# loicmagne/tinynerf

Measured on AMD Instinct MI355X. Metric: ray-samples/sec (K-Planes training step: sampler + render fwd + bwd + Adam), higher is better.
Workload: dtype f32 (f16x2-split products)

## Files before the change

### tinynerf_amd/csrc/kplanes.hip

```cpp
#include "kplanes_scatter.h"
#include <algorithm>

namespace {

using tn::f32x4k;

struct KpArgs {
    int n_scales, C;
    int H[TN_KPLANES_MAX_SCALES], W[TN_KPLANES_MAX_SCALES];
    const float *planes[TN_KPLANES_MAX_SCALES][3];
    float *grads[TN_KPLANES_MAX_SCALES][3];
};

template <int NV>
__global__ __launch_bounds__(256) void kplanes_fwd_kernel(KpArgs a, const float *__restrict__ x, int64_t x_stride,
                                                          int64_t n, float *__restrict__ feat)
{
    const int lane = tn::lane_id(), j = lane & 31, h = lane >> 5;
    const int64_t n_tiles = (n + 31) >> 5;
    const int C = a.C, FD = a.n_scales * C;
    for (int64_t tile = (int64_t)blockIdx.x * 4 + (threadIdx.x >> 6); tile < n_tiles; tile += (int64_t)gridDim.x * 4) {
        const int64_t row = tile * 32 + j;
        if (row >= n) continue;
        const float xs[3] = {x[row * x_stride], x[row * x_stride + 1], x[row * x_stride + 2]};
        for (int s = 0; s < a.n_scales; ++s) {
            f32x4k prod[NV];
#pragma unroll
            for (int q = 0; q < NV; ++q) prod[q] = f32x4k{1.f, 1.f, 1.f, 1.f};
#pragma unroll
            for (int p = 0; p < 3; ++p) {
                if (a.planes[s][p] == nullptr) continue;
                float u, v;
                tn::pair_uv(xs, p, u, v);
                const tn::PlaneTaps t = tn::plane_taps(u, v, a.H[s], a.W[s], C);
                f32x4k val[NV];
                tn::plane_gather<NV>(a.planes[s][p], t, h * (C / 2), val);
#pragma unroll
                for (int q = 0; q < NV; ++q) prod[q] = prod[q] * val[q];
            }
            f32x4k *o = reinterpret_cast<f32x4k *>(feat + row * FD + s * C + h * (C / 2));
#pragma unroll
            for (int q = 0; q < NV; ++q) o[q] = prod[q];
        }
    }
}

template <int NV>
__global__ __launch_bounds__(256, 3) void kplanes_bwd_kernel(KpArgs a, const float *__restrict__ x, int64_t x_stride,
                                                          int64_t n, const float *__restrict__ grad_feat)
{
    __shared__ __attribute__((aligned(16))) float lds[4 * tn::KP_WAVE_LDS];
    const int lane = tn::lane_id(), j = lane & 31, h = lane >> 5;
    float *wave_lds = lds + (threadIdx.x >> 6) * tn::KP_WAVE_LDS;
    const int64_t n_tiles = (n + 31) >> 5;
    const int C = a.C, FD = a.n_scales * C;
    for (int64_t tile = (int64_t)blockIdx.x * 4 + (threadIdx.x >> 6); tile < n_tiles; tile += (int64_t)gridDim.x * 4) {
        const int64_t row = tile * 32 + j;
        const bool valid = row < n;
        const int64_t rr = valid ? row : 0;
        const float xs[3] = {x[rr * x_stride], x[rr * x_stride + 1], x[rr * x_stride + 2]};
        for (int s = 0; s < a.n_scales; ++s) {
            f32x4k g[NV];
#pragma unroll
            for (int q = 0; q < NV; ++q)
                g[q] = valid ? reinterpret_cast<const f32x4k *>(grad_feat + row * FD + s * C + h * (C / 2))[q]
                             : f32x4k{0.f, 0.f, 0.f, 0.f};
            const float *const pl[3] = {a.planes[s][0], a.planes[s][1], a.planes[s][2]};
            float *const gr[3] = {a.grads[s][0], a.grads[s][1], a.grads[s][2]};
            tn::kp_scatter_scale<NV, 4>(pl, gr, a.H[s], a.W[s], C, xs, valid, g, h * (C / 2), wave_lds, j, h);
        }
    }
}

int make_args(const tn_kplanes_desc *d, KpArgs &a, float *const (*grads)[3])
{
    TN_REQUIRE(d, TN_E_NULL, "kplanes: null descriptor");
    TN_REQUIRE(d->n_scales >= 1 && d->n_scales <= TN_KPLANES_MAX_SCALES, TN_E_CONFIG, "kplanes: n_scales out of range");
    TN_REQUIRE(d->channels == 8 || d->channels == 16 || d->channels == 32, TN_E_CONFIG, "kplanes: channels must be 8, 16 or 32");
    a.n_scales = d->n_scales; a.C = d->channels;
    for (int s = 0; s < d->n_scales; ++s) {
        TN_REQUIRE(d->height[s] > 0 && d->width[s] > 0, TN_E_SIZE, "kplanes: bad plane resolution");
        TN_REQUIRE((int64_t)d->height[s] * d->width[s] * d->channels < (1ll << 30), TN_E_SIZE, "kplanes: plane too large (2^30 elements)");
        a.H[s] = d->height[s]; a.W[s] = d->width[s];
        TN_REQUIRE(d->planes[s][0], TN_E_NULL, "kplanes: null plane pointer");
        for (int p = 0; p < 3; ++p) {
            TN_REQUIRE(((uintptr_t)d->planes[s][p] & 15) == 0, TN_E_ALIGN, "kplanes: planes must be 16-byte aligned");
            a.planes[s][p] = d->planes[s][p];
            a.grads[s][p] = nullptr;
            if (grads && d->planes[s][p]) {
                TN_REQUIRE(grads[s][p], TN_E_NULL, "kplanes: null grad plane pointer");
                a.grads[s][p] = grads[s][p];
            }
        }
    }
    return TN_OK;
}

template <int ACT>
__device__ __forceinline__ float bd_act(float v)
{
    if (ACT == TN_ACT_EXP_M1) return expf(v - 1.0f);
    if (ACT == TN_ACT_EXP) return expf(v);
    if (ACT == TN_ACT_SIGMOID) return 1.0f / (1.0f + expf(-v));
    return v;
}

template <int ACT>
__global__ __launch_bounds__(256) void basis_dot_fwd_kernel(const float *__restrict__ f, const float *__restrict__ basis, int64_t n, int C,
                                                            int K, float *__restrict__ out)
{
    const int lane = tn::lane_id();
    const int64_t wave = ((int64_t)blockIdx.x * blockDim.x + threadIdx.x) >> 6, n_waves = ((int64_t)gridDim.x * blockDim.x) >> 6;
    for (int64_t i = wave; i < n; i += n_waves) {
        const float *fi = f + i * C, *bi = basis + i * (int64_t)K * C;
        for (int k = 0; k < K; ++k) {
            float acc = 0.0f;
            for (int c = lane; c < C; c += 64) acc += fi[c] * bi[k * C + c];
            acc = tn::wave_sum(acc);
            if (lane == 0) out[i * K + k] = bd_act<ACT>(acc);
        }
    }
}

template <int ACT>
__global__ __launch_bounds__(256) void basis_dot_bwd_kernel(const float *__restrict__ f, const float *__restrict__ basis,
                                                            const float *__restrict__ g_out, int64_t n, int C, int K,
                                                            float *__restrict__ g_f, float *__restrict__ g_basis, int accumulate_f)
{
    const int lane = tn::lane_id();
    const int64_t wave = ((int64_t)blockIdx.x * blockDim.x + threadIdx.x) >> 6, n_waves = ((int64_t)gridDim.x * blockDim.x) >> 6;
    for (int64_t i = wave; i < n; i += n_waves) {
        const float *fi = f + i * C, *bi = basis + i * (int64_t)K * C;
        float gv[4];
        for (int k = 0; k < K; ++k) {
            float acc = 0.0f;
            for (int c = lane; c < C; c += 64) acc += fi[c] * bi[k * C + c];
            acc = tn::wave_sum(acc);
            const float g = g_out[i * K + k];
            if (ACT == TN_ACT_EXP_M1) gv[k] = g * expf(fminf(fmaxf(acc - 1.0f, -15.0f), 15.0f));
            else if (ACT == TN_ACT_EXP) gv[k] = g * expf(fminf(fmaxf(acc, -15.0f), 15.0f));
            else if (ACT == TN_ACT_SIGMOID) { const float y = 1.0f / (1.0f + expf(-acc)); gv[k] = g * y * (1.0f - y); }
            else gv[k] = g;
        }
        for (int c = lane; c < C; c += 64) {
            const float fc = fi[c];
            float a = accumulate_f ? g_f[i * C + c] : 0.0f;
            for (int k = 0; k < K; ++k) {
                a += gv[k] * bi[k * C + c];
                if (g_basis) g_basis[(i * K + k) * C + c] = gv[k] * fc;
            }
            g_f[i * C + c] = a;
        }
    }
}

inline unsigned tile_blocks(int64_t n) { return (unsigned)std::min<int64_t>(((n + 31) / 32 + 3) / 4, 256 * 8); }

}

extern "C" int tn_kplanes_fwd(const tn_kplanes_desc *desc, const float *x, int64_t x_stride, int64_t n, float *feat,
                              void *stream)
{
    KpArgs a;
    if (int rc = make_args(desc, a, nullptr)) return rc;
    TN_REQUIRE(n >= 0 && x_stride >= 3, TN_E_SIZE, "tn_kplanes_fwd: bad size");
    if (n == 0) return TN_OK;
    TN_REQUIRE(x && feat, TN_E_NULL, "tn_kplanes_fwd: null pointer");
    TN_REQUIRE(((uintptr_t)feat & 15) == 0, TN_E_ALIGN, "tn_kplanes_fwd: feat must be 16-byte aligned");
    hipStream_t s = (hipStream_t)stream;
    const dim3 grid(tile_blocks(n)), block(256);
    switch (a.C) {
    case 8: kplanes_fwd_kernel<1><<<grid, block, 0, s>>>(a, x, x_stride, n, feat); break;
    case 16: kplanes_fwd_kernel<2><<<grid, block, 0, s>>>(a, x, x_stride, n, feat); break;
    default: kplanes_fwd_kernel<4><<<grid, block, 0, s>>>(a, x, x_stride, n, feat); break;
    }
    return tn::check_launch("kplanes_fwd_kernel");
}

extern "C" int tn_kplanes_bwd(const tn_kplanes_desc *desc, const float *x, int64_t x_stride, int64_t n,
                              const float *grad_feat, float *const (*grad_planes)[3], void *stream)
{
    KpArgs a;
    TN_REQUIRE(grad_planes, TN_E_NULL, "tn_kplanes_bwd: null grad_planes");
    if (int rc = make_args(desc, a, grad_planes)) return rc;
    TN_REQUIRE(n >= 0 && x_stride >= 3, TN_E_SIZE, "tn_kplanes_bwd: bad size");
    if (n == 0) return TN_OK;
    TN_REQUIRE(x && grad_feat, TN_E_NULL, "tn_kplanes_bwd: null pointer");
    TN_REQUIRE(((uintptr_t)grad_feat & 15) == 0, TN_E_ALIGN, "tn_kplanes_bwd: grad_feat must be 16-byte aligned");
    hipStream_t s = (hipStream_t)stream;
    const dim3 grid(tile_blocks(n)), block(256);
    switch (a.C) {
    case 8: kplanes_bwd_kernel<1><<<grid, block, 0, s>>>(a, x, x_stride, n, grad_feat); break;
    case 16: kplanes_bwd_kernel<2><<<grid, block, 0, s>>>(a, x, x_stride, n, grad_feat); break;
    default: kplanes_bwd_kernel<4><<<grid, block, 0, s>>>(a, x, x_stride, n, grad_feat); break;
    }
    return tn::check_launch("kplanes_bwd_kernel");
}

extern "C" int tn_basis_dot_fwd(const float *f, const float *basis, int64_t n, int32_t channels, int32_t n_out, int32_t activation,
                                float *out, void *stream)
{
    TN_REQUIRE(n >= 0 && channels > 0 && n_out >= 1 && n_out <= 4, TN_E_SIZE, "tn_basis_dot_fwd: bad size (1 <= n_out <= 4)");
    if (n == 0) return TN_OK;
    TN_REQUIRE(f && basis && out, TN_E_NULL, "tn_basis_dot_fwd: null pointer");
    const dim3 grid((unsigned)std::min<int64_t>((n + 3) / 4, 256 * 8)), block(256);
    hipStream_t s = (hipStream_t)stream;
    switch (activation) {
    case TN_ACT_EXP_M1: basis_dot_fwd_kernel<TN_ACT_EXP_M1><<<grid, block, 0, s>>>(f, basis, n, channels, n_out, out); break;
    case TN_ACT_SIGMOID: basis_dot_fwd_kernel<TN_ACT_SIGMOID><<<grid, block, 0, s>>>(f, basis, n, channels, n_out, out); break;
    case TN_ACT_EXP: basis_dot_fwd_kernel<TN_ACT_EXP><<<grid, block, 0, s>>>(f, basis, n, channels, n_out, out); break;
    case TN_ACT_NONE: basis_dot_fwd_kernel<TN_ACT_NONE><<<grid, block, 0, s>>>(f, basis, n, channels, n_out, out); break;
    default: return tn::fail(TN_E_CONFIG, "tn_basis_dot_fwd: unknown activation");
    }
    return tn::check_launch("basis_dot_fwd_kernel");
}

extern "C" int tn_basis_dot_bwd(const float *f, const float *basis, const float *grad_out, int64_t n, int32_t channels, int32_t n_out,
                                int32_t activation, float *grad_f, float *grad_basis, int32_t accumulate_f, void *stream)
{
    TN_REQUIRE(n >= 0 && channels > 0 && n_out >= 1 && n_out <= 4, TN_E_SIZE, "tn_basis_dot_bwd: bad size (1 <= n_out <= 4)");
    if (n == 0) return TN_OK;
    TN_REQUIRE(f && basis && grad_out && grad_f, TN_E_NULL, "tn_basis_dot_bwd: null pointer");
    const dim3 grid((unsigned)std::min<int64_t>((n + 3) / 4, 256 * 8)), block(256);
    hipStream_t s = (hipStream_t)stream;
    switch (activation) {
    case TN_ACT_EXP_M1: basis_dot_bwd_kernel<TN_ACT_EXP_M1><<<grid, block, 0, s>>>(f, basis, grad_out, n, channels, n_out, grad_f, grad_basis, accumulate_f); break;
    case TN_ACT_SIGMOID: basis_dot_bwd_kernel<TN_ACT_SIGMOID><<<grid, block, 0, s>>>(f, basis, grad_out, n, channels, n_out, grad_f, grad_basis, accumulate_f); break;
    case TN_ACT_EXP: basis_dot_bwd_kernel<TN_ACT_EXP><<<grid, block, 0, s>>>(f, basis, grad_out, n, channels, n_out, grad_f, grad_basis, accumulate_f); break;
    case TN_ACT_NONE: basis_dot_bwd_kernel<TN_ACT_NONE><<<grid, block, 0, s>>>(f, basis, grad_out, n, channels, n_out, grad_f, grad_basis, accumulate_f); break;
    default: return tn::fail(TN_E_CONFIG, "tn_basis_dot_bwd: unknown activation");
    }
    return tn::check_launch("basis_dot_bwd_kernel");
}
```

### tinynerf_amd/csrc/kplanes_scatter.h

```cpp
#pragma once
#include "kplanes_device.h"

#ifdef TN_PHASE_TIMERS
extern __device__ unsigned long long tn_phase_cycles_b[16];
#endif
namespace tn {

constexpr int KP_GS = 36;
constexpr int KP_WAVE_LDS = 32 * KP_GS + 2 * 4 * 32;

template <int NV, int CS>
__device__ __forceinline__ void kp_scatter_scale(const float *const (&planes)[3], float *const (&grads)[3], int H, int W, int C,
                                                 const float (&xs)[3], bool valid, const f32x4k (&g)[NV], int c0,
                                                 float *__restrict__ wave_lds, int j, int h)
{
#ifdef TN_PHASE_TIMERS
    unsigned long long pts_ = __builtin_amdgcn_s_memtime();
#define TN_PTS(k) { __builtin_amdgcn_sched_barrier(0); const unsigned long long n_ = __builtin_amdgcn_s_memtime(); if (tn::lane_id() == 0) atomicAdd(&tn_phase_cycles_b[k], n_ - pts_); pts_ = __builtin_amdgcn_s_memtime(); __builtin_amdgcn_sched_barrier(0); }
#endif
    float *tileG = wave_lds;
    int *tileO = reinterpret_cast<int *>(tileG + 32 * KP_GS);
    float *tileW = tileG + 32 * KP_GS + 4 * 32;
    PlaneTaps t[3];
    f32x4k val[3][NV];
#pragma unroll
    for (int p = 0; p < 3; ++p) {
        float u, v;
        pair_uv(xs, p, u, v);
        t[p] = plane_taps(u, v, H, W, C);
        if (planes[p]) {
            plane_gather<NV, CS>(planes[p], t[p], c0, val[p]);
            __builtin_amdgcn_sched_barrier(0);
        } else {
#pragma unroll
            for (int q = 0; q < NV; ++q) val[p][q] = f32x4k{1.f, 1.f, 1.f, 1.f};
        }
    }
#ifdef TN_PHASE_TIMERS
    TN_PTS(8)
#endif
#pragma unroll
    for (int p = 0; p < 3; ++p) {
        if (grads[p] == nullptr) continue;
#pragma unroll
        for (int q = 0; q < NV; ++q) {
            const f32x4k gp = p == 0 ? g[q] * val[1][q] * val[2][q]
                                     : (p == 1 ? g[q] * val[0][q] * val[2][q] : g[q] * (val[0][q] * val[1][q]));
            *reinterpret_cast<f32x4k *>(tileG + j * KP_GS + c0 + CS * q) = gp;
        }
#pragma unroll
        for (int k = 0; k < 2; ++k) {
            const int o = h ? t[p].off[2 + k] : t[p].off[0 + k];
            const float w = h ? t[p].w[2 + k] : t[p].w[0 + k];
            const bool live = valid && o >= 0;
            tileO[(2 * h + k) * 32 + j] = live ? 4 * o : 0;
            tileW[(2 * h + k) * 32 + j] = live ? w : 0.0f;
        }
        const int cell = valid ? t[p].cell : -1 - j;
        const int next_cell = __shfl_down(cell, 1, 64);
        const int dcell = (j < 31) ? next_cell - cell : 0x40000000;
        const int rowlen = W + 4;
        const unsigned run_end = (unsigned)__ballot(dcell != 0);
        const unsigned mv_xp = (unsigned)__ballot(dcell == 1), mv_xm = (unsigned)__ballot(dcell == -1);
        const unsigned mv_yp = (unsigned)__ballot(dcell == rowlen), mv_ym = (unsigned)__ballot(dcell == -rowlen);
        const unsigned mv_pp = (unsigned)__ballot(dcell == rowlen + 1), mv_mp = (unsigned)__ballot(dcell == rowlen - 1);
        const unsigned mv_pm = (unsigned)__ballot(dcell == -rowlen + 1), mv_mm = (unsigned)__ballot(dcell == -rowlen - 1);
        const unsigned mv_diag = mv_pp | mv_mp | mv_pm | mv_mm;
        asm volatile("" ::: "memory");
#ifdef TN_PHASE_TIMERS
        TN_PTS(9)
#endif
        const int c = j;
        char *const gplane = reinterpret_cast<char *>(grads[p]);
        const unsigned c4 = 4u * (unsigned)c;
        auto add_at = [&](unsigned byte_off, float v) { atomicAdd(reinterpret_cast<float *>(gplane + byte_off), v); };
        if (c < C) {
            const int4 *O0 = reinterpret_cast<const int4 *>(tileO + (2 * h) * 32), *O1 = O0 + 8;
            const f32x4k *W0 = reinterpret_cast<const f32x4k *>(tileW + (2 * h) * 32);
            const f32x4k *W1 = W0 + 8;
            float a0 = 0.0f, a1 = 0.0f;
#pragma clang loop unroll(disable)
            for (int s4 = 0; s4 < 8; ++s4) {
                const f32x4k w0 = W0[s4], w1 = W1[s4];
                const int4 o0v = O0[s4], o1v = O1[s4];
                const int o0a[4] = {o0v.x, o0v.y, o0v.z, o0v.w}, o1a[4] = {o1v.x, o1v.y, o1v.z, o1v.w};
                float gv[4];
#pragma unroll
                for (int u = 0; u < 4; ++u) gv[u] = tileG[(4 * s4 + u) * KP_GS + c];
#pragma unroll
                for (int u = 0; u < 4; ++u) {
                    const int sI = 4 * s4 + u;
                    a0 = fmaf(gv[u], w0[u], a0);
                    a1 = fmaf(gv[u], w1[u], a1);
                    if ((run_end >> sI) & 1u) {
                        const unsigned o0 = (unsigned)o0a[u] + c4, o1 = (unsigned)o1a[u] + c4;
                        if ((mv_xp >> sI) & 1u) {
                            add_at(o0, a0);
                            a0 = a1; a1 = 0.0f;
                        } else if ((mv_xm >> sI) & 1u) {
                            add_at(o1, a1);
                            a1 = a0; a0 = 0.0f;
                        } else if ((mv_yp >> sI) & 1u) {
                            const float t0 = __shfl_xor(a0, 32, 64), t1 = __shfl_xor(a1, 32, 64);
                            if (h == 0) {
                                add_at(o0, a0);
                                add_at(o1, a1);
                            }
                            a0 = h == 0 ? t0 : 0.0f; a1 = h == 0 ? t1 : 0.0f;
                        } else if ((mv_ym >> sI) & 1u) {
                            const float t0 = __shfl_xor(a0, 32, 64), t1 = __shfl_xor(a1, 32, 64);
                            if (h == 1) {
                                add_at(o0, a0);
                                add_at(o1, a1);
                            }
                            a0 = h == 1 ? t0 : 0.0f; a1 = h == 1 ? t1 : 0.0f;
                        } else if ((mv_diag >> sI) & 1u) {
                            const float t0 = __shfl_xor(a0, 32, 64), t1 = __shfl_xor(a1, 32, 64);
                            if ((mv_pp >> sI) & 1u) {
                                add_at(o0, a0);
                                if (h == 0) add_at(o1, a1);
                                a0 = h == 0 ? t1 : 0.0f; a1 = 0.0f;
                            } else if ((mv_mp >> sI) & 1u) {
                                add_at(o1, a1);
                                if (h == 0) add_at(o0, a0);
                                a1 = h == 0 ? t0 : 0.0f; a0 = 0.0f;
                            } else if ((mv_pm >> sI) & 1u) {
                                add_at(o0, a0);
                                if (h == 1) add_at(o1, a1);
                                a0 = h == 1 ? t1 : 0.0f; a1 = 0.0f;
                            } else {
                                add_at(o1, a1);
                                if (h == 1) add_at(o0, a0);
                                a1 = h == 1 ? t0 : 0.0f; a0 = 0.0f;
                            }
                        } else {
                            add_at(o0, a0);
                            add_at(o1, a1);
                            a0 = 0.0f; a1 = 0.0f;
                        }
                    }
                }
            }
        }
        asm volatile("" ::: "memory");
#ifdef TN_PHASE_TIMERS
        TN_PTS(10)
#endif
    }
}

}
```

### tinynerf_amd/csrc/mlp_bwd2.hip

```cpp
#include "mlp_stage.h"
#include "kplanes_scatter.h"
#include <algorithm>
#include <type_traits>

extern "C" int64_t tn_mlp_bwd_layers_workspace_bytes(const tn_mlp_desc *desc, int64_t n);
extern "C" int tn_mlp_bwd_layers(const tn_mlp_desc *desc, const float *x, const float *aux, const float *grad_y, int64_t n,
                                 float *const *grad_weights, float *const *grad_biases, float *grad_x, float *workspace, void *stream);
extern "C" int tn_mlp_wgrad_rows2(const float *g_rows, int64_t g_stride, const float *g_rows2, int64_t g_stride2, const float *a_rows,
                                  int64_t a_stride, int na, float *gW, int ldw, int col0, float *gB, float *gW2, int ldw2, int col02,
                                  float *gB2, int64_t n, void *stream);
extern "C" int tn_heads_dx_rows(const float *w_a, int ld_a, int col0_a, const float *w_b, int ld_b, int col0_b, const float *g_a, int64_t gs_a,
                                const float *g_b, int64_t gs_b, int F, float *out, int64_t out_stride, const void *mask, int64_t mask_stride,
                                int64_t n, void *stream);
extern "C" int tn_mlp_wgrad_lean_pair(const tn_mlp_desc *desc, const tn_mlp_desc *partner, const float *x, const float *aux, int64_t n,
                                      float *const *gw, float *const *gb, float *const *gws, float *const *gbs, const float *ws_a,
                                      const float *ws_b, void *stream);
extern "C" int tn_mlp_wgrad_lean_check(const tn_mlp_desc *desc, const tn_mlp_desc *partner, const float *x, const float *aux, int64_t n,
                                       float *const *gw, float *const *gb, float *const *gws, float *const *gbs, const float *ws_a,
                                       const float *ws_b);
extern "C" int tn_mlp_wgrad_rows(const float *g_rows, int64_t g_stride, int ng, const float *a_rows, int64_t a_stride, int na, float *gW,
                                 int ldw, int col0, int kmax, float *gB, int64_t n, void *stream);

#ifdef TN_PHASE_TIMERS
__device__ unsigned long long tn_phase_cycles_b[16];
#define TN_PTB_BEGIN unsigned long long ptb_ = __builtin_amdgcn_s_memtime();
#define TN_PTB(k) { __builtin_amdgcn_sched_barrier(0); const unsigned long long n_ = __builtin_amdgcn_s_memtime(); if (tn::lane_id() == 0) atomicAdd(&tn_phase_cycles_b[k], n_ - ptb_); ptb_ = __builtin_amdgcn_s_memtime(); __builtin_amdgcn_sched_barrier(0); }
extern "C" int tn_debug_phase_cycles_b(unsigned long long *out, int reset) {
    hipMemcpyFromSymbol(out, HIP_SYMBOL(tn_phase_cycles_b), sizeof(unsigned long long) * 16);
    if (reset) { unsigned long long z[16] = {}; hipMemcpyToSymbol(HIP_SYMBOL(tn_phase_cycles_b), z, sizeof(z)); }
    return 0;
}
#else
#define TN_PTB_BEGIN
#define TN_PTB(k)
#endif
namespace {

using tn::f32x16;
using tn::f32x4;
using namespace tn::mlp;

template <int N, class F>
__device__ __forceinline__ void static_for(F &&f) {
    if constexpr (N > 0) {
        static_for<N - 1>(f);
        f(std::integral_constant<int, N - 1>{});
    }
}

__device__ __forceinline__ float act_grad(float pre, int act) {
    if (act == TN_ACT_EXP_M1) return expf(fminf(fmaxf(pre - 1.0f, -15.0f), 15.0f));
    if (act == TN_ACT_SIGMOID) { const float s = 1.0f / (1.0f + expf(-pre)); return s * (1.0f - s); }
    return 1.0f;
}

struct PairArgs { MlpArgs b; const float *gy; float *stash; int64_t g0_stride = 0; };

struct KpBwd {
    int H[3], W[3];
    const float *planes[3][3];
    float *grads[3][3];
    const float *coords;
    int64_t coord_stride;
};

template <int H>
__device__ __forceinline__ void first_dgrad(const float *__restrict__ Wf, int sf, int out, const float (&gp)[4],
                                            const unsigned (&mask)[H / 32], int h, f32x16 (&G)[H / 32])
{
#pragma unroll
    for (int kb = 0; kb < H / 32; ++kb) {
#pragma unroll
        for (int q = 0; q < 4; ++q) {
            f32x4 acc4 = {0.f, 0.f, 0.f, 0.f};
#pragma unroll
            for (int o = 0; o < 4; ++o) {
                if (o < out) {
                    const f32x4 w = *reinterpret_cast<const f32x4 *>(Wf + o * sf + 32 * kb + 8 * q + 4 * h);
                    acc4 += w * gp[o];
                }
            }
#pragma unroll
            for (int u = 0; u < 4; ++u) G[kb][4 * q + u] = mask_keep(acc4[u], mask[kb], 4 * q + u);
        }
    }
}

template <int H, int NH, int WPB, bool STASHED, bool ACCUM = false, bool PAIR = false, bool KP = false, bool G0B = false>
__global__ __launch_bounds__(WPB * 64) void mlp_chain_kernel(MlpArgs a, const float *__restrict__ x, const float *__restrict__ aux,
                                                             const float *__restrict__ gy, int64_t n, float *__restrict__ gx,
                                                             float *__restrict__ stash, PairArgs pr, KpBwd kp)
{
    static_assert(!KP || (STASHED && PAIR && !ACCUM && H == 64), "the fused scatter belongs to the paired, stashed chain of the width-64 heads");
    static_assert(!G0B || (STASHED && !PAIR && !KP && !ACCUM), "G0B: another head's G_0 rows join a stashed, unpaired chain's grad_x");
    extern __shared__ __attribute__((aligned(16))) float lds[];
    constexpr int T = H / 32;
    constexpr int L = NH + 1;
    stage_weights(a, lds);
    const float *ldsb = lds + a.lds_floats;
    if constexpr (PAIR || G0B) stage_weights(pr.b, lds + a.lds_floats);
    __syncthreads();
    if constexpr (STASHED && NH > 1) {
        constexpr int sl = H + 4;
        for (int l = 1; l < NH; ++l) {
            float *W = lds + a.w_off[l];
            for (int e = threadIdx.x; e < H * H; e += blockDim.x) {
                const int r = e / H, c = e - r * H;
                if (r < c) { const float t = W[r * sl + c]; W[r * sl + c] = W[c * sl + r]; W[c * sl + r] = t; }
            }
        }
        __syncthreads();
    }
    const int lane = tn::lane_id(), j_ = lane & 31, h_ = lane >> 5;
    const int wave = __builtin_amdgcn_readfirstlane(threadIdx.x >> 6);
    const int64_t n_tiles = (n + 31) >> 5;
    const int G0 = a.K0_pad >> 3;
    const int out = a.out_dim;

    unsigned nmask[NH][T];
    float npre[4], ngy[4];
    unsigned bmask[T];
    float bpre[4], bgy[4];
    const int Rb = stash_rows(H, 1, 0);
    const int extra_ = extra_rows(a.enc, a.in_dim, a.K0_pad);
    auto fetch_tile = [&](int64_t t) {
        if constexpr (PAIR) {
            const float *qb = pr.stash + t * (int64_t)(Rb * 32) + stash_rows_w(H, 1, 0) * 32;
            const unsigned *mb = reinterpret_cast<const unsigned *>(qb + 4 * 32);
#pragma unroll
            for (int ob = 0; ob < T; ++ob) bmask[ob] = mb[ob * 64 + lane];
            int64_t rb = t * 32 + j_;
            rb = rb < n ? rb : n - 1;
            const int outb = pr.b.out_dim;
#pragma unroll
            for (int o = 0; o < 4; ++o) {
                const int oc = o < outb ? o : outb - 1;
                bpre[o] = qb[oc * 32 + j_];
                bgy[o] = pr.gy[rb * outb + oc];
            }
        }
        const float *q = stash + t * (int64_t)(stash_rows(H, NH, extra_) * 32) + stash_rows_w(H, NH, extra_) * 32;
        const unsigned *mm = reinterpret_cast<const unsigned *>(q + 4 * 32);
#pragma unroll
        for (int l = 0; l < NH; ++l)
#pragma unroll
            for (int ob = 0; ob < T; ++ob) nmask[l][ob] = mm[(l * T + ob) * 64 + lane];
        int64_t r = t * 32 + j_;
        r = r < n ? r : n - 1;
#pragma unroll
        for (int o = 0; o < 4; ++o) {
            const int oc = o < out ? o : out - 1;
            npre[o] = q[oc * 32 + j_];
            ngy[o] = gy[r * out + oc];
        }
    };
    if constexpr (STASHED) {
        const int64_t t0 = (int64_t)blockIdx.x * WPB + wave;
        fetch_tile(t0 < n_tiles ? t0 : n_tiles - 1);
    }

    for (int64_t tile = (int64_t)blockIdx.x * WPB + wave; tile < n_tiles; tile += (int64_t)gridDim.x * WPB) {
        int j = j_, h = h_;
        asm volatile("" : "+v"(j), "+v"(h));
        TN_PTB_BEGIN
        const int64_t row = tile * 32 + j;
        const bool valid = row < n;
        const int extra = extra_rows(a.enc, a.in_dim, a.K0_pad);
        float *st = stash + tile * (int64_t)(stash_rows(H, NH, extra) * 32);
        float *stH = st;
        float *stG = st + NH * H * 32;
        float *stP = st + 2 * NH * H * 32;
        float *stE = stP + 4 * 32;
        float *stQ = st + stash_rows_w(H, NH, extra) * 32;
        unsigned *stM = reinterpret_cast<unsigned *>(stQ + 4 * 32);
        const float *Wf = lds + a.w_off[L - 1];
        const float *Bf = lds + a.b_off[L - 1];
        const int sf = a.stride[L - 1];
        unsigned mask[NH][T];
        float gp[4];
        unsigned pmask[T];
        float gpb[4];
        if constexpr (STASHED) {
#pragma unroll
            for (int l = 0; l < NH; ++l)
#pragma unroll
                for (int ob = 0; ob < T; ++ob) mask[l][ob] = nmask[l][ob];
#pragma unroll
            for (int o = 0; o < 4; ++o) gp[o] = (valid && o < out) ? ngy[o] * act_grad(npre[o], a.out_act) : 0.0f;
            if constexpr (PAIR) {
#pragma unroll
                for (int ob = 0; ob < T; ++ob) pmask[ob] = bmask[ob];
#pragma unroll
                for (int o = 0; o < 4; ++o) gpb[o] = (valid && o < pr.b.out_dim) ? bgy[o] * act_grad(bpre[o], pr.b.out_act) : 0.0f;
            }
            {
                const int64_t tn_ = tile + (int64_t)gridDim.x * WPB;
                fetch_tile(tn_ < n_tiles ? tn_ : n_tiles - 1);
            }
            if constexpr (PAIR) {
                float *stb = pr.stash + tile * (int64_t)(Rb * 32);
#pragma unroll
                for (int o = 0; o < 4; ++o)
                    if (h == 0) stb[(2 * H + o) * 32 + j] = gpb[o];
                f32x16 Gb[T];
                first_dgrad<H>(ldsb + pr.b.w_off[1], pr.b.stride[1], pr.b.out_dim, gpb, pmask, h, Gb);
#pragma unroll
                for (int ob = 0; ob < T; ++ob) store_rows(stb + H * 32, Gb[ob], ob, j, h);
            }
#pragma unroll
            for (int o = 0; o < 4; ++o)
                if (h == 0) stP[o * 32 + j] = gp[o];
            (void)stQ; (void)stM;
        } else {
        const float *xrow = x + (valid ? row : 0) * a.in_dim;
        float aux3[3] = {0.f, 0.f, 0.f};
        const float *auxrow = nullptr;
        if (valid) {
            if (a.enc == TN_ENC_POSENC) { aux3[0] = xrow[0]; aux3[1] = xrow[1]; aux3[2] = xrow[2]; }
            else if (a.enc == TN_ENC_DIR_CAT) { aux3[0] = aux[3 * row]; aux3[1] = aux[3 * row + 1]; aux3[2] = aux[3 * row + 2]; }
            else if (a.enc == TN_ENC_AUX_CAT) auxrow = aux + (int64_t)(a.aux_index ? a.aux_index[row] : row) * a.aux_stride;
        }
        const int xs = x_slots(a.enc, a.in_dim);

        f32x16 act[T];
        {
            const float *W0 = lds + a.w_off[0];
#pragma unroll
            for (int ob = 0; ob < T; ++ob) act[ob] = tn::bias_tile(lds + a.b_off[0], ob, h);
            f32x4 b = fetch_input(a, xrow, aux3, valid, 0, h, auxrow);
            for (int g = 0; g < G0; ++g) {
                f32x4 bn = {0.f, 0.f, 0.f, 0.f};
                if (g + 1 < G0) bn = fetch_input(a, xrow, aux3, valid, g + 1, h, auxrow);
                f32x4 w[T];
#pragma unroll
                for (int ob = 0; ob < T; ++ob) w[ob] = load_a4<true>(W0, 32 * ob + j, 8 * g + 4 * h, a.K0, a.stride[0]);
#pragma unroll
                for (int u = 0; u < 4; ++u)
#pragma unroll
                    for (int ob = 0; ob < T; ++ob) act[ob] = tn::mfma32(w[ob][u], b[u], act[ob]);
                if (extra > 0 && 8 * g + 4 * h + 3 >= xs) {
#pragma unroll
                    for (int u = 0; u < 4; ++u) {
                        const int q = 8 * g + 4 * h + u;
                        if (q >= xs) stE[(q - xs) * 32 + j] = b[u];
                    }
                }
                b = bn;
            }
#pragma unroll
            for (int ob = 0; ob < T; ++ob) {
                tn::pin16(act[ob]);
                act[ob] = tn::relu16(act[ob]);
                mask[0][ob] = relu_bits(act[ob]);
                store_rows(stH, act[ob], ob, j, h);
            }
        }
        static_for<NH - 1>([&](auto lc) {
            constexpr int l = decltype(lc)::value + 1;
            tn::hidden_layer<H>(lds + a.w_off[l], lds + a.b_off[l], a.stride[l], act, j, h);
#pragma unroll
            for (int ob = 0; ob < T; ++ob) {
                mask[l][ob] = relu_bits(act[ob]);
                store_rows(stH + l * H * 32, act[ob], ob, j, h);
            }
        });

#pragma unroll
        for (int o = 0; o < 4; ++o) {
            gp[o] = 0.0f;
            if (o < out) {
                const float pre = tn::small_out<H>(Wf + o * sf, Bf[o], act, h);
                gp[o] = valid ? gy[row * out + o] * act_grad(pre, a.out_act) : 0.0f;
            }
            if (h == 0) stP[o * 32 + j] = gp[o];
        }
        }
        TN_PTB(0)
        f32x16 G[T];
#pragma unroll
        for (int kb = 0; kb < T; ++kb) {
// ... 530 lines not shown
            const int nn = 32 * tn_ + (r & 3) + 8 * (r >> 2) + 4 * h;
            if (kok && nn < Nl) atomicAdd(&a.gW[l][(int64_t)nn * Kl + kc], acc[m][r]);
        }
        if (tkm == 0) {
            float sum = dbacc[m];
            sum += __shfl_xor(sum, 32, 64);
            const int nn = 32 * tn_ + i;
            if (h == 0 && nn < Nl) atomicAdd(&a.gB[l][nn], sum);
        }
    }
}

struct WgradPlan { int R, Rt, xs, aw, chunks; size_t lds; };
WgradPlan wgrad_plan(int enc, int in_dim, int K0_pad, int H, int NH, bool x_elsewhere = false) {
    WgradPlan p;
    const int extra = extra_rows(enc, in_dim, K0_pad);
    p.R = stash_rows_w(H, NH, extra); p.Rt = stash_rows(H, NH, extra);
    p.xs = x_elsewhere ? 0 : x_slots(enc, in_dim);
    p.aw = enc == TN_ENC_AUX_CAT ? K0_pad - in_dim : 0;
    p.chunks = p.R * 8 + (p.xs > 0 ? 8 * in_dim : 0);
    p.lds = ((size_t)p.R * 36 + (p.xs > 0 ? 32 * (size_t)in_dim : 0) + 32 * (size_t)p.aw) * 4;
    return p;
}

MlpArgs compact_first_layer(const MlpArgs &a)
{
    MlpArgs c = a;
    const int H = a.N[0];
    c.K0_pad = (a.in_dim + 7) & ~7;
    int off = 0;
    for (int l = 0; l < a.n_layers; ++l) {
        const int Kp = l == 0 ? c.K0_pad : H;
        const int rows = (l == a.n_layers - 1) ? (a.out_dim <= 4 ? a.out_dim : ((a.out_dim + 31) & ~31)) : H;
        c.stride[l] = Kp + 4;
        c.w_off[l] = off; off += rows * c.stride[l];
        c.b_off[l] = off; off += (rows + 3) & ~3;
    }
    c.lds_floats = off;
    return c;
}

MlpArgs first_layer_only(const MlpArgs &a)
{
    MlpArgs c = compact_first_layer(a);
    c.n_layers = 1;
    c.lds_floats = c.b_off[0] + ((a.N[0] + 3) & ~3);
    return c;
}

int launch_chain_g0b(const MlpArgs &b, const MlpArgs &a, const float *x, const float *gy_b, int64_t n, float *gx, float *stash_b,
                     const float *g0_rows_a, int64_t g0_stride_a, hipStream_t s)
{
    constexpr int WPS = 8;
    PairArgs pr;
    pr.b = first_layer_only(a); pr.gy = nullptr; pr.stash = const_cast<float *>(g0_rows_a); pr.g0_stride = g0_stride_a;
    const size_t lds_bytes = ((size_t)b.lds_floats + (size_t)pr.b.lds_floats) * 4;
    return launch(mlp_chain_kernel<64, 1, WPS, true, false, false, false, true>, WPS, lds_bytes, grid_per_cu(n, WPS, lds_bytes), s,
                  "mlp_chain_kernel(g0b)", b, x, nullptr, gy_b, n, gx, stash_b, pr, KpBwd());
}

int64_t tile_floats(const MlpArgs &m) { return (int64_t)stash_rows(64, m.n_layers - 1, extra_rows(m.enc, m.in_dim, m.K0_pad)) * 32; }
int64_t g0_floats(const MlpArgs &m) { return (int64_t)(m.n_layers - 1) * 64 * 32; }

bool x_cols_from_rows(const MlpArgs &a, bool stashed) {
    return stashed && a.x_rows != nullptr && (a.in_dim == 128 || a.in_dim == 256) && x_slots(a.enc, a.in_dim) == a.in_dim;
}
bool x_cols_from_rows2(const MlpArgs &a, const MlpArgs &b) {
    return x_cols_from_rows(a, true) && b.x_rows == a.x_rows && b.x_rows_stride == a.x_rows_stride && extra_rows(a.enc, a.in_dim, a.K0_pad) == 0;
}

template <int H, int NH>
int launch_chain(const MlpArgs &a, const float *x, const float *aux, const float *gy, int64_t n, float *gx, float *stash, bool stashed,
                 hipStream_t s, const PairArgs *pair = nullptr, const KpBwd *kpb = nullptr)
{
    if (kpb) {
        if constexpr (H == 64 && NH == 4) {
            if (!(pair && stashed && a.enc == TN_ENC_AUX_CAT && a.in_dim == 96)) return tn::fail(TN_E_CONFIG, "mlp_bwd: fused scatter needs the paired K-Planes heads");
            constexpr int WPK = 8;
            const MlpArgs ac = compact_first_layer(a);
            PairArgs pr = *pair;
            pr.b = compact_first_layer(pair->b);
            const size_t lds_bytes = ((size_t)ac.lds_floats + (size_t)pr.b.lds_floats + (size_t)WPK * tn::KP_WAVE_LDS) * 4;
            if (lds_bytes > (size_t)LDS_LIMIT_BYTES) return tn::fail(TN_E_CONFIG, "mlp_bwd: weights + scatter tiles do not fit LDS");
            return launch(mlp_chain_kernel<H, NH, WPK, true, false, true, true>, WPK, lds_bytes, grid_blocks(n, WPK, 256), s,
                          "mlp_chain_kernel(kplanes)", ac, x, aux, gy, n, gx, stash, pr, *kpb);
        } else return tn::fail(TN_E_CONFIG, "mlp_bwd: fused scatter is built for the 5-layer colour head");
    }
    size_t lds_bytes = (size_t)a.lds_floats * 4;
    constexpr int WPB = 8;
    constexpr int WPS = NH == 1 ? 10 : 16;
    constexpr int WPP = 8;
    int wpb = stashed ? WPS : WPB;
    auto kern = stashed ? mlp_chain_kernel<H, NH, WPS, true> : mlp_chain_kernel<H, NH, WPB, false>;
    if (stashed && a.accum_gx && (gx != nullptr || a.gx_rows != nullptr) && a.enc != TN_ENC_POSENC && (a.in_dim & 31) == 0) kern = mlp_chain_kernel<H, NH, WPS, true, true>;
    PairArgs pr;
    pr.gy = nullptr; pr.stash = nullptr;
    if (pair) {
        pr = *pair;
        if constexpr (NH == 4) kern = mlp_chain_kernel<H, NH, WPP, true, false, true>;
        else return tn::fail(TN_E_CONFIG, "mlp_bwd: the paired chain is built for the 5-layer colour head");
        wpb = WPP;
        lds_bytes += (size_t)pr.b.lds_floats * 4;
    } else pr.b = a;
    if (lds_bytes > (size_t)LDS_LIMIT_BYTES) return tn::fail(TN_E_CONFIG, "mlp_bwd: weights do not fit LDS");
    return launch(kern, wpb, lds_bytes, grid_per_cu(n, wpb, lds_bytes), s, "mlp_chain_kernel", a, x, aux, gy, n, gx, stash, pr, KpBwd());
}

int chain(const MlpArgs &a, const float *x, const float *aux, const float *gy, int64_t n, float *gx, float *stash, bool stashed,
          hipStream_t s, const PairArgs *pair = nullptr, const KpBwd *kpb = nullptr)
{
    return a.n_layers == 2 ? launch_chain<64, 1>(a, x, aux, gy, n, gx, stash, stashed, s, pair, kpb)
                           : launch_chain<64, 4>(a, x, aux, gy, n, gx, stash, stashed, s, pair, kpb);
}

using WgradKern = decltype(&mlp_wgrad_kernel<64, 1, 1, 8, 4, false>);

struct WgradStep {
    WgradArgs w;
    bool rows;
    WgradKern kern;
    int waves;
    size_t lds;
    int64_t blocks;
    const char *what;
};

template <int H, int NH>
int plan_wgrad(WgradStep &st, const MlpArgs &a, float *const *gw, float *const *gb, int64_t n, bool stashed)
{
    WgradArgs &w = st.w;
    constexpr int T = H / 32;
    w.n_layers = a.n_layers; w.in_dim = a.in_dim; w.K0 = a.K0; w.K0_pad = a.K0_pad; w.enc = a.enc; w.n_freqs = a.n_freqs;
    w.out_dim = a.out_dim;
    w.Tk0 = (a.K0_pad + 31) / 32;
    for (int l = 0; l < a.n_layers; ++l) { w.gW[l] = gw[l]; w.gB[l] = gb[l]; w.K[l] = a.K[l]; w.N[l] = a.N[l]; }
    w.aux_index = a.aux_index; w.aux_stride = a.aux_stride;
    st.rows = x_cols_from_rows(a, stashed);
    w.tk_skip = st.rows ? a.in_dim / 32 : 0;
    w.total_tiles = T * (w.Tk0 - w.tk_skip) + (NH - 1) * T * T + T;
    const WgradPlan wp = wgrad_plan(a.enc, a.in_dim, a.K0_pad, H, NH, st.rows);
    if (wp.lds > (size_t)LDS_LIMIT_BYTES) return tn::fail(TN_E_CONFIG, "mlp_bwd: workspace tile does not fit LDS");
    if (wp.xs > 0 && (a.in_dim & 3)) return tn::fail(TN_E_CONFIG, "mlp_bwd: in_dim must be a multiple of 4");
    const bool aux = a.enc == TN_ENC_AUX_CAT;
    st.what = "mlp_wgrad_kernel";
    if (extra_rows(a.enc, a.in_dim, a.K0_pad) == 0 && (wp.xs > 0 || (st.rows && aux)) && NH >= 2) {
        if constexpr (H == 64 && NH >= 2) {
            constexpr int RG4 = H + NH * H + 4;
            const int xw4 = st.rows ? 0 : a.in_dim;
            st.lds = 2 * ((size_t)RG4 * RS + 32 * (size_t)xw4 + 32 * (size_t)wp.aw) * 4 + 32 * 16;
            if (st.lds <= (size_t)LDS_LIMIT_BYTES && w.Tk0 - w.tk_skip + (NH - 1) * 2 + 1 <= 12 && RG4 * 8 + 8 * xw4 <= 5 * 768) {
                st.kern = aux ? mlp_wgrad4_kernel<NH, 12, 5, true> : mlp_wgrad4_kernel<NH, 12, 5, false>;
                st.waves = 12; st.blocks = grid_blocks(n, 1, 256); st.what = "mlp_wgrad4_kernel";
                return TN_OK;
            }
        }
    }
    struct Tiling { int max_tiles, max_chunks; WgradKern kern; int waves; };
    const Tiling tilings[] = {
        {8, 4 * 512, mlp_wgrad_kernel<H, NH, 1, 8, 4, false>, 8},    {16, 4 * 1024, mlp_wgrad_kernel<H, NH, 1, 16, 4, false>, 16},
        {24, 7 * 768, mlp_wgrad_kernel<H, NH, 2, 12, 7, false>, 12}, {32, 6 * 1024, mlp_wgrad_kernel<H, NH, 2, 16, 6, false>, 16},
        {48, 10 * 1024, mlp_wgrad_kernel<H, NH, 3, 16, 10, false>, 16}};
    st.lds = wp.lds; st.blocks = grid_blocks(n, 1, 256 * (wp.lds * 2 <= (size_t)LDS_LIMIT_BYTES ? 2 : 1));
    if (aux) {
        if constexpr (NH == 4) {
            if (st.rows && w.total_tiles <= 24 && wp.chunks <= 7 * 768 && wp.aw <= 64) {
                st.kern = mlp_wgrad_kernel<H, NH, 2, 12, 7, true>; st.waves = 12; st.what = "mlp_wgrad_kernel(aux)";
                return TN_OK;
// ... 203 lines not shown
```

Before: 343.9 million.

## Assign contiguous tile spans per wave and carry scatter runs across tiles

```diff
diff --git a/tinynerf_amd/csrc/kplanes.hip b/tinynerf_amd/csrc/kplanes.hip
--- a/tinynerf_amd/csrc/kplanes.hip
+++ b/tinynerf_amd/csrc/kplanes.hip
@@ -45,16 +45,22 @@
     }
 }
 
+constexpr int KP_BWD_MIN_SPAN = 4;
 template <int NV>
 __global__ __launch_bounds__(256, 3) void kplanes_bwd_kernel(KpArgs a, const float *__restrict__ x, int64_t x_stride,
                                                           int64_t n, const float *__restrict__ grad_feat)
 {
-    __shared__ __attribute__((aligned(16))) float lds[4 * tn::KP_WAVE_LDS];
+    constexpr int CARRY = TN_KPLANES_MAX_SCALES * 3 * tn::KP_CARRY_PLANE;
+    __shared__ __attribute__((aligned(16))) float lds[4 * (tn::KP_WAVE_LDS + CARRY)];
     const int lane = tn::lane_id(), j = lane & 31, h = lane >> 5;
-    float *wave_lds = lds + (threadIdx.x >> 6) * tn::KP_WAVE_LDS;
+    const int wave = __builtin_amdgcn_readfirstlane(threadIdx.x >> 6);
+    float *wave_lds = lds + wave * tn::KP_WAVE_LDS;
+    float *carry = lds + 4 * tn::KP_WAVE_LDS + wave * CARRY;
     const int64_t n_tiles = (n + 31) >> 5;
     const int C = a.C, FD = a.n_scales * C;
-    for (int64_t tile = (int64_t)blockIdx.x * 4 + (threadIdx.x >> 6); tile < n_tiles; tile += (int64_t)gridDim.x * 4) {
+    int64_t tile_begin, tile_end;
+    tn::kp_wave_span(n_tiles, (int64_t)blockIdx.x * 4 + wave, (int64_t)gridDim.x * 4, KP_BWD_MIN_SPAN, tile_begin, tile_end);
+    for (int64_t tile = tile_begin; tile < tile_end; ++tile) {
         const int64_t row = tile * 32 + j;
         const bool valid = row < n;
         const int64_t rr = valid ? row : 0;
@@ -67,7 +73,8 @@
                              : f32x4k{0.f, 0.f, 0.f, 0.f};
             const float *const pl[3] = {a.planes[s][0], a.planes[s][1], a.planes[s][2]};
             float *const gr[3] = {a.grads[s][0], a.grads[s][1], a.grads[s][2]};
-            tn::kp_scatter_scale<NV, 4>(pl, gr, a.H[s], a.W[s], C, xs, valid, g, h * (C / 2), wave_lds, j, h);
+            tn::kp_scatter_scale<NV, 4, true>(pl, gr, a.H[s], a.W[s], C, xs, valid, g, h * (C / 2), wave_lds, j, h,
+                                              carry + s * 3 * tn::KP_CARRY_PLANE, tile > tile_begin, tile + 1 < tile_end);
         }
     }
 }
@@ -155,6 +162,7 @@
 }
 
 inline unsigned tile_blocks(int64_t n) { return (unsigned)std::min<int64_t>(((n + 31) / 32 + 3) / 4, 256 * 8); }
+inline unsigned span_blocks(int64_t n) { return (unsigned)((tn::kp_span_waves((n + 31) / 32, 4 * 256 * 8, KP_BWD_MIN_SPAN) + 3) / 4); }
 
 }
 
@@ -188,7 +196,7 @@
     TN_REQUIRE(x && grad_feat, TN_E_NULL, "tn_kplanes_bwd: null pointer");
     TN_REQUIRE(((uintptr_t)grad_feat & 15) == 0, TN_E_ALIGN, "tn_kplanes_bwd: grad_feat must be 16-byte aligned");
     hipStream_t s = (hipStream_t)stream;
-    const dim3 grid(tile_blocks(n)), block(256);
+    const dim3 grid(span_blocks(n)), block(256);
     switch (a.C) {
     case 8: kplanes_bwd_kernel<1><<<grid, block, 0, s>>>(a, x, x_stride, n, grad_feat); break;
     case 16: kplanes_bwd_kernel<2><<<grid, block, 0, s>>>(a, x, x_stride, n, grad_feat); break;
diff --git a/tinynerf_amd/csrc/kplanes_scatter.h b/tinynerf_amd/csrc/kplanes_scatter.h
--- a/tinynerf_amd/csrc/kplanes_scatter.h
+++ b/tinynerf_amd/csrc/kplanes_scatter.h
@@ -8,11 +8,25 @@
 
 constexpr int KP_GS = 36;
 constexpr int KP_WAVE_LDS = 32 * KP_GS + 2 * 4 * 32;
+constexpr int KP_CARRY_PLANE = 2 * 64 + 5;
 
-template <int NV, int CS>
+__device__ __host__ inline int64_t kp_span_waves(int64_t n_tiles, int64_t n_waves, int min_span) {
+    const int64_t want = n_tiles / min_span > 1 ? n_tiles / min_span : 1;
+    return want < n_waves ? want : n_waves;
+}
+__device__ __forceinline__ void kp_wave_span(int64_t n_tiles, int64_t gw, int64_t n_waves, int min_span, int64_t &begin, int64_t &end) {
+    const int64_t act = kp_span_waves(n_tiles, n_waves, min_span);
+    begin = gw < act ? gw * n_tiles / act : n_tiles;
+    end = gw < act ? (gw + 1) * n_tiles / act : n_tiles;
+}
+
+struct KpMoves { unsigned end, xp, xm, yp, ym, pp, mp, pm, mm, diag; };
+
+template <int NV, int CS, bool CARRY = false>
 __device__ __forceinline__ void kp_scatter_scale(const float *const (&planes)[3], float *const (&grads)[3], int H, int W, int C,
                                                  const float (&xs)[3], bool valid, const f32x4k (&g)[NV], int c0,
-                                                 float *__restrict__ wave_lds, int j, int h)
+                                                 float *__restrict__ wave_lds, int j, int h, float *__restrict__ carry = nullptr,
+                                                 bool have = false, bool keep = false)
 {
 #ifdef TN_PHASE_TIMERS
     unsigned long long pts_ = __builtin_amdgcn_s_memtime();
@@ -58,14 +72,16 @@
         }
         const int cell = valid ? t[p].cell : -1 - j;
         const int next_cell = __shfl_down(cell, 1, 64);
-        const int dcell = (j < 31) ? next_cell - cell : 0x40000000;
+        const int dcell = (j < 31) ? next_cell - cell : ((CARRY && keep) ? 0 : 0x40000000);
         const int rowlen = W + 4;
-        const unsigned run_end = (unsigned)__ballot(dcell != 0);
-        const unsigned mv_xp = (unsigned)__ballot(dcell == 1), mv_xm = (unsigned)__ballot(dcell == -1);
-        const unsigned mv_yp = (unsigned)__ballot(dcell == rowlen), mv_ym = (unsigned)__ballot(dcell == -rowlen);
-        const unsigned mv_pp = (unsigned)__ballot(dcell == rowlen + 1), mv_mp = (unsigned)__ballot(dcell == rowlen - 1);
-        const unsigned mv_pm = (unsigned)__ballot(dcell == -rowlen + 1), mv_mm = (unsigned)__ballot(dcell == -rowlen - 1);
-        const unsigned mv_diag = mv_pp | mv_mp | mv_pm | mv_mm;
+        KpMoves mv;
+        mv.end = (unsigned)__ballot(dcell != 0);
+        mv.xp = (unsigned)__ballot(dcell == 1); mv.xm = (unsigned)__ballot(dcell == -1);
+        mv.yp = (unsigned)__ballot(dcell == rowlen); mv.ym = (unsigned)__ballot(dcell == -rowlen);
+        mv.pp = (unsigned)__ballot(dcell == rowlen + 1); mv.mp = (unsigned)__ballot(dcell == rowlen - 1);
+        mv.pm = (unsigned)__ballot(dcell == -rowlen + 1); mv.mm = (unsigned)__ballot(dcell == -rowlen - 1);
+        mv.diag = mv.pp | mv.mp | mv.pm | mv.mm;
+        const int cell_first = __builtin_amdgcn_readfirstlane(cell), cell_last = __builtin_amdgcn_readlane(cell, 31);
         asm volatile("" ::: "memory");
 #ifdef TN_PHASE_TIMERS
         TN_PTS(9)
@@ -79,6 +95,67 @@
             const f32x4k *W0 = reinterpret_cast<const f32x4k *>(tileW + (2 * h) * 32);
             const f32x4k *W1 = W0 + 8;
             float a0 = 0.0f, a1 = 0.0f;
+            auto close_run = [&](const KpMoves &m, int sI, unsigned o0, unsigned o1) {
+                if ((m.xp >> sI) & 1u) {
+                    add_at(o0, a0);
+                    a0 = a1; a1 = 0.0f;
+                } else if ((m.xm >> sI) & 1u) {
+                    add_at(o1, a1);
+                    a1 = a0; a0 = 0.0f;
+                } else if ((m.yp >> sI) & 1u) {
+                    const float t0 = __shfl_xor(a0, 32, 64), t1 = __shfl_xor(a1, 32, 64);
+                    if (h == 0) {
+                        add_at(o0, a0);
+                        add_at(o1, a1);
+                    }
+                    a0 = h == 0 ? t0 : 0.0f; a1 = h == 0 ? t1 : 0.0f;
+                } else if ((m.ym >> sI) & 1u) {
+                    const float t0 = __shfl_xor(a0, 32, 64), t1 = __shfl_xor(a1, 32, 64);
+                    if (h == 1) {
+                        add_at(o0, a0);
+                        add_at(o1, a1);
+                    }
+                    a0 = h == 1 ? t0 : 0.0f; a1 = h == 1 ? t1 : 0.0f;
+                } else if ((m.diag >> sI) & 1u) {
+                    const float t0 = __shfl_xor(a0, 32, 64), t1 = __shfl_xor(a1, 32, 64);
+                    if ((m.pp >> sI) & 1u) {
+                        add_at(o0, a0);
+                        if (h == 0) add_at(o1, a1);
+                        a0 = h == 0 ? t1 : 0.0f; a1 = 0.0f;
+                    } else if ((m.mp >> sI) & 1u) {
+                        add_at(o1, a1);
+                        if (h == 0) add_at(o0, a0);
+                        a1 = h == 0 ? t0 : 0.0f; a0 = 0.0f;
+                    } else if ((m.pm >> sI) & 1u) {
+                        add_at(o0, a0);
+                        if (h == 1) add_at(o1, a1);
+                        a0 = h == 1 ? t1 : 0.0f; a1 = 0.0f;
+                    } else {
+                        add_at(o1, a1);
+                        if (h == 1) add_at(o0, a0);
+                        a1 = h == 1 ? t0 : 0.0f; a0 = 0.0f;
+                    }
+                } else {
+                    add_at(o0, a0);
+                    add_at(o1, a1);
+                    a0 = 0.0f; a1 = 0.0f;
+                }
+            };
+            float *const slot = carry + p * KP_CARRY_PLANE;
+            int *const slot_i = reinterpret_cast<int *>(slot) + 128;
+            if constexpr (CARRY) {
+                if (have) {
+                    a0 = slot[32 * h + c]; a1 = slot[64 + 32 * h + c];
+                    const int d = cell_first - __builtin_amdgcn_readfirstlane(slot_i[0]);
+                    if (d != 0) {
+                        KpMoves m;
+                        m.xp = d == 1; m.xm = d == -1; m.yp = d == rowlen; m.ym = d == -rowlen;
+                        m.pp = d == rowlen + 1; m.mp = d == rowlen - 1; m.pm = d == -rowlen + 1; m.mm = d == -rowlen - 1;
+                        m.diag = m.pp | m.mp | m.pm | m.mm;
+                        close_run(m, 0, (unsigned)slot_i[1 + 2 * h] + c4, (unsigned)slot_i[2 + 2 * h] + c4);
+                    }
+                }
+            }
 #pragma clang loop unroll(disable)
             for (int s4 = 0; s4 < 8; ++s4) {
                 const f32x4k w0 = W0[s4], w1 = W1[s4];
@@ -92,53 +169,14 @@
                     const int sI = 4 * s4 + u;
                     a0 = fmaf(gv[u], w0[u], a0);
                     a1 = fmaf(gv[u], w1[u], a1);
-                    if ((run_end >> sI) & 1u) {
-                        const unsigned o0 = (unsigned)o0a[u] + c4, o1 = (unsigned)o1a[u] + c4;
-                        if ((mv_xp >> sI) & 1u) {
-                            add_at(o0, a0);
-                            a0 = a1; a1 = 0.0f;
-                        } else if ((mv_xm >> sI) & 1u) {
-                            add_at(o1, a1);
-                            a1 = a0; a0 = 0.0f;
-                        } else if ((mv_yp >> sI) & 1u) {
-                            const float t0 = __shfl_xor(a0, 32, 64), t1 = __shfl_xor(a1, 32, 64);
-                            if (h == 0) {
-                                add_at(o0, a0);
-                                add_at(o1, a1);
-                            }
-                            a0 = h == 0 ? t0 : 0.0f; a1 = h == 0 ? t1 : 0.0f;
-                        } else if ((mv_ym >> sI) & 1u) {
-                            const float t0 = __shfl_xor(a0, 32, 64), t1 = __shfl_xor(a1, 32, 64);
-                            if (h == 1) {
-                                add_at(o0, a0);
-                                add_at(o1, a1);
-                            }
-                            a0 = h == 1 ? t0 : 0.0f; a1 = h == 1 ? t1 : 0.0f;
-                        } else if ((mv_diag >> sI) & 1u) {
-                            const float t0 = __shfl_xor(a0, 32, 64), t1 = __shfl_xor(a1, 32, 64);
-                            if ((mv_pp >> sI) & 1u) {
-                                add_at(o0, a0);
-                                if (h == 0) add_at(o1, a1);
-                                a0 = h == 0 ? t1 : 0.0f; a1 = 0.0f;
-                            } else if ((mv_mp >> sI) & 1u) {
-                                add_at(o1, a1);
-                                if (h == 0) add_at(o0, a0);
-                                a1 = h == 0 ? t0 : 0.0f; a0 = 0.0f;
-                            } else if ((mv_pm >> sI) & 1u) {
-                                add_at(o0, a0);
-                                if (h == 1) add_at(o1, a1);
-                                a0 = h == 1 ? t1 : 0.0f; a1 = 0.0f;
-                            } else {
-                                add_at(o1, a1);
-                                if (h == 1) add_at(o0, a0);
-                                a1 = h == 1 ? t0 : 0.0f; a0 = 0.0f;
-                            }
-                        } else {
-                            add_at(o0, a0);
-                            add_at(o1, a1);
-                            a0 = 0.0f; a1 = 0.0f;
-                        }
-                    }
+                    if ((mv.end >> sI) & 1u) close_run(mv, sI, (unsigned)o0a[u] + c4, (unsigned)o1a[u] + c4);
+                }
+            }
+            if constexpr (CARRY) {
+                if (keep) {
+                    slot[32 * h + c] = a0; slot[64 + 32 * h + c] = a1;
+                    if (h == 0 && c == 0) slot_i[0] = cell_last;
+                    if (h == 0 && c < 4) slot_i[1 + c] = tileO[c * 32 + 31];
                 }
             }
         }
diff --git a/tinynerf_amd/csrc/mlp_bwd2.hip b/tinynerf_amd/csrc/mlp_bwd2.hip
--- a/tinynerf_amd/csrc/mlp_bwd2.hip
+++ b/tinynerf_amd/csrc/mlp_bwd2.hip
@@ -56,6 +56,7 @@
 
 struct PairArgs { MlpArgs b; const float *gy; float *stash; int64_t g0_stride = 0; };
 
+constexpr int KP_CHAIN_MIN_SPAN = 2;
 struct KpBwd {
     int H[3], W[3];
     const float *planes[3][3];
@@ -154,12 +155,14 @@
             ngy[o] = gy[r * out + oc];
         }
     };
-    if constexpr (STASHED) {
-        const int64_t t0 = (int64_t)blockIdx.x * WPB + wave;
-        fetch_tile(t0 < n_tiles ? t0 : n_tiles - 1);
-    }
-
-    for (int64_t tile = (int64_t)blockIdx.x * WPB + wave; tile < n_tiles; tile += (int64_t)gridDim.x * WPB) {
+    int64_t tile_begin = (int64_t)blockIdx.x * WPB + wave, tile_end = n_tiles, tile_step = (int64_t)gridDim.x * WPB;
+    if constexpr (KP) {
+        tn::kp_wave_span(n_tiles, tile_begin, tile_step, KP_CHAIN_MIN_SPAN, tile_begin, tile_end);
+        tile_step = 1;
+    }
+    if constexpr (STASHED) fetch_tile(tile_begin < tile_end ? tile_begin : n_tiles - 1);
+
+    for (int64_t tile = tile_begin; tile < tile_end; tile += tile_step) {
         int j = j_, h = h_;
         asm volatile("" : "+v"(j), "+v"(h));
         TN_PTB_BEGIN
@@ -194,8 +197,8 @@
                 for (int o = 0; o < 4; ++o) gpb[o] = (valid && o < pr.b.out_dim) ? bgy[o] * act_grad(bpre[o], pr.b.out_act) : 0.0f;
             }
             {
-                const int64_t tn_ = tile + (int64_t)gridDim.x * WPB;
-                fetch_tile(tn_ < n_tiles ? tn_ : n_tiles - 1);
+                const int64_t tn_ = tile + tile_step;
+                fetch_tile(tn_ < tile_end ? tn_ : n_tiles - 1);
             }
             if constexpr (PAIR) {
                 float *stb = pr.stash + tile * (int64_t)(Rb * 32);
@@ -892,7 +895,8 @@
             pr.b = compact_first_layer(pair->b);
             const size_t lds_bytes = ((size_t)ac.lds_floats + (size_t)pr.b.lds_floats + (size_t)WPK * tn::KP_WAVE_LDS) * 4;
             if (lds_bytes > (size_t)LDS_LIMIT_BYTES) return tn::fail(TN_E_CONFIG, "mlp_bwd: weights + scatter tiles do not fit LDS");
-            return launch(mlp_chain_kernel<H, NH, WPK, true, false, true, true>, WPK, lds_bytes, grid_blocks(n, WPK, 256), s,
+            const int64_t span_waves = tn::kp_span_waves((n + 31) / 32, 256 * WPK, KP_CHAIN_MIN_SPAN);
+            return launch(mlp_chain_kernel<H, NH, WPK, true, false, true, true>, WPK, lds_bytes, (span_waves + WPK - 1) / WPK, s,
                           "mlp_chain_kernel(kplanes)", ac, x, aux, gy, n, gx, stash, pr, *kpb);
         } else return tn::fail(TN_E_CONFIG, "mlp_bwd: fused scatter is built for the 5-layer colour head");
     }
```

After: 342.7 million, median of 2. No clear change (-0.4%).
